# hyrise/hyrise

Hardware: AMD Instinct MI355X
Metric: rows/sec TableScan+JoinHash, TPC-H SF10 lineitem (higher is better)
Workload: dtype u16

## Files before the change

hyrise_amd/csrc/join.hip:

```cpp
#include "hy_device.hpp"
#include "hy_decode.hpp"
#include "hy_arithmetic.hpp"
#include "hy_scan_job.hpp"

#include <algorithm>
#include <atomic>
#include <cmath>
#include <chrono>
#include <cstring>
#include <type_traits>

namespace hy {

constexpr uint32_t JOIN_TILE = 4096;
constexpr uint32_t JOIN_THREADS = 512;
constexpr uint32_t JOIN_WAVES = JOIN_THREADS / 64;
constexpr uint32_t JOIN_WAVE_ROWS = JOIN_TILE / JOIN_WAVES;
constexpr uint32_t JOIN_ROUNDS = JOIN_WAVE_ROWS / 64;
constexpr uint32_t JOIN_STAGE = JOIN_TILE + 256;
constexpr uint32_t MAX_PARTITIONS = 256;
typedef uint32_t u32x2_t __attribute__((ext_vector_type(2)));
typedef uint32_t u32x4_t __attribute__((ext_vector_type(4)));
constexpr uint32_t PROBE_SIZE_PER_CHUNK = 65535u * 2u;
constexpr uint32_t BLOOM_BITS = 1u << 20;
// ... 2171 lines not shown

static void free_zeroed_blocks() {
  for (ZeroedBlocks& z : t_zeroed) {
    if (z.table) (void)hipFree(z.table);
    if (z.filter) (void)hipFree(z.filter);
    z = ZeroedBlocks{};
  }
}

void release_thread_join_state() {
  if (t_mailbox) (void)hipHostFree(t_mailbox);
  t_mailbox = t_mailbox_dev = nullptr;
  free_zeroed_blocks();
}

static hy_status join_mailbox(JoinMailbox** host, JoinMailbox** device) {
  if (!t_mailbox) {
    static_assert(sizeof(JoinMailbox) <= 256, "the mailbox is a 256-byte pinned block");
    HY_HIP(hipHostMalloc(reinterpret_cast<void**>(&t_mailbox), 256, hipHostMallocMapped));
    HY_HIP(hipHostGetDevicePointer(reinterpret_cast<void**>(&t_mailbox_dev), t_mailbox, 0));
  }
  std::memset(t_mailbox, 0, sizeof(JoinMailbox));
  *host = t_mailbox;
  *device = t_mailbox_dev;
  return HY_OK;
}

template <uint32_t WIDTH> struct FillGroup { static constexpr uint32_t ROWS = WIDTH == 4 ? 4 : 8; };
template <uint32_t WIDTH>
__device__ __forceinline__ void load_group_words(const SliceView& view, uint32_t first, uint32_t (&word)[FillGroup<WIDTH>::ROWS]) {
  const char* base = static_cast<const char*>(view.data);
  if constexpr (WIDTH == 4) {
    const u32x4_t v = *reinterpret_cast<const u32x4_t*>(base + size_t{first} * 4);
    word[0] = v.x; word[1] = v.y; word[2] = v.z; word[3] = v.w;
  } else if constexpr (WIDTH == 2) {
    const u32x4_t v = *reinterpret_cast<const u32x4_t*>(base + size_t{first} * 2);
    const uint32_t w[4] = {v.x, v.y, v.z, v.w};
#pragma unroll
    for (uint32_t j = 0; j < 8; ++j) word[j] = (w[j / 2] >> (16 * (j & 1))) & 0xFFFFu;
  } else {
    const u32x2_t v = *reinterpret_cast<const u32x2_t*>(base + first);
    const uint32_t w[2] = {v.x, v.y};
#pragma unroll
    for (uint32_t j = 0; j < 8; ++j) word[j] = (w[j / 4] >> (8 * (j & 3))) & 0xFFu;
  }
}

__device__ __forceinline__ int32_t view_key(const SliceView& view, uint32_t row) {
  if (view.kind == VIEW_INT32) return static_cast<const int32_t*>(view.data)[row];
  const uint32_t stored = view.kind == VIEW_FOR8 ? static_cast<const uint8_t*>(view.data)[row] : view.kind == VIEW_FOR16 ? static_cast<const uint16_t*>(view.data)[row] : static_cast<const uint32_t*>(view.data)[row];
  return static_cast<int32_t>(stored + static_cast<uint32_t>(static_cast<const int32_t*>(view.aux)[row / HY_FOR_BLOCK_SIZE]));
}

template <uint32_t WIDTH>
struct FillWords {
  static constexpr uint32_t GROUP = FillGroup<WIDTH>::ROWS, GROUPS = SLICE_ROWS / 256 / GROUP;
  uint32_t word[GROUPS][GROUP];
  int32_t front[GROUPS];
  uint32_t bias[GROUPS];
  int32_t key_before;
  bool has_before;
};

template <uint32_t WIDTH>
__device__ __forceinline__ void load_fill_words(const MaterializeArgs& a, const SliceView& view, uint32_t slice_index, uint32_t tid, FillWords<WIDTH>& w) {
  constexpr uint32_t GROUP = FillWords<WIDTH>::GROUP, GROUPS = FillWords<WIDTH>::GROUPS;
  const uint32_t row_count = view.row_count, lane = tid & 63;
#pragma unroll
  for (uint32_t i = 0; i < GROUPS; ++i) {
    const uint32_t first = (i * 256 + tid) * GROUP;
    load_group_words<WIDTH>(view, view.row_begin + (first < row_count ? first : 0), w.word[i]);
    w.front[i] = 0;
    if (lane == 0 && first > 0 && first < row_count) w.front[i] = view_key(view, view.row_begin + first - 1);
    w.bias[i] = view.kind == VIEW_INT32 ? 0u : static_cast<uint32_t>(static_cast<const int32_t*>(view.aux)[(view.row_begin + (first < row_count ? first : 0)) / HY_FOR_BLOCK_SIZE]);
  }
  w.key_before = 0;
  w.has_before = false;
  if (tid == 0) {
    for (uint32_t before = slice_index; before-- > 0;) {
      const SliceView earlier = a.views[before];
      if (earlier.row_count == 0) continue;
      w.key_before = view_key(earlier, earlier.row_begin + earlier.row_count - 1);
      w.has_before = true;
      break;
    }
  }
}

template <uint32_t WIDTH>
__device__ __forceinline__ void fill_checked_process(const MaterializeArgs& a, const SliceView& view, const FillWords<WIDTH>& w, uint32_t origin, uint32_t range, u32x2_entry_t* entries,
                                                     uint32_t* s_bits, uint32_t* s_base, int32_t* s_extent, uint32_t tid, int32_t* low_out, int32_t* high_out, uint32_t* flags_out) {
  constexpr uint32_t GROUP = FillGroup<WIDTH>::ROWS, GROUPS = SLICE_ROWS / 256 / GROUP;
  const uint32_t row_count = view.row_count, lane = tid & 63, wave = tid >> 6;
  const auto& word = w.word;
  int32_t front[GROUPS];
#pragma unroll
  for (uint32_t i = 0; i < GROUPS; ++i) front[i] = w.front[i];
  const int32_t key_before = w.key_before;
  const bool has_before = w.has_before;
  int32_t low = 0x7FFFFFFF, high = static_cast<int32_t>(0x80000000u);
  int32_t key[GROUPS][GROUP];
#pragma unroll
  for (uint32_t i = 0; i < GROUPS; ++i) {
    const uint32_t first = (i * 256 + tid) * GROUP;
    const uint32_t bias = w.bias[i];
#pragma unroll
// ... 125 lines not shown
  uint64_t low = ~0ull, high = 0, bits = 0;
  for (uint32_t i = tid; i < a.n_slices; i += 256) {
    uint64_t* record = partials + 4 * size_t{i};
    const uint64_t record_low = __hip_atomic_load(record + 0, __ATOMIC_RELAXED, __HIP_MEMORY_SCOPE_AGENT), record_high = __hip_atomic_load(record + 1, __ATOMIC_RELAXED, __HIP_MEMORY_SCOPE_AGENT);
    low = record_low < low ? record_low : low;
    high = record_high > high ? record_high : high;
    bits |= __hip_atomic_load(record + 2, __ATOMIC_RELAXED, __HIP_MEMORY_SCOPE_AGENT);
  }
#pragma unroll
  for (int d = 32; d > 0; d >>= 1) {
    bits |= __shfl_xor(bits, d, 64);
    const uint64_t other_low = __shfl_xor(low, d, 64), other_high = __shfl_xor(high, d, 64);
    low = other_low < low ? other_low : low;
    high = other_high > high ? other_high : high;
  }
  __syncthreads();
  if ((tid & 63) == 0) { s_min[tid >> 6] = low; s_max[tid >> 6] = high; atomicOr(&s_flags, static_cast<uint32_t>(bits)); }
  __syncthreads();
  if (tid != 0) return;
  for (uint32_t w = 0; w < 4; ++w) { low = s_min[w] < low ? s_min[w] : low; high = s_max[w] > high ? s_max[w] : high; }
  verdict->key_min = low ^ SIGN;
  verdict->key_max = high ^ SIGN;
  verdict->unsorted_signed = s_flags & 1u ? 1 : 0;
  verdict->equal_neighbours = s_flags & 2u ? 1 : 0;
  verdict->outside_hint = s_flags & 4u ? 1 : 0;
  verdict->done = 1;
  __threadfence_system();
}

constexpr uint32_t FW_STEP = 512;
constexpr uint32_t FW_STEPS_PER_SLICE = SLICE_ROWS / FW_STEP;
constexpr uint32_t FW_WINDOW = 2048;
static_assert(HY_FOR_BLOCK_SIZE % FW_STEP == 0, "a step lies in one FrameOfReference block");

constexpr uint32_t FW_BATCH = 4;

struct FillWaveState {
  uint64_t unsorted = 0, equal = 0, outside = 0;
  int32_t low = 0x7FFFFFFF, high = static_cast<int32_t>(0x80000000u);
  bool any_rows = false;
  int32_t carry = 0;
  bool has_carry = false;
};

template <uint32_t WIDTH>
__device__ __forceinline__ int32_t fill_step_key(const u32x4_t& a, const u32x4_t& b, uint32_t bias, uint32_t j) {
  uint32_t stored;
  if constexpr (WIDTH == 4) stored = j < 4 ? a[j] : b[j - 4];
  else if constexpr (WIDTH == 2) stored = (a[j / 2] >> (16 * (j & 1))) & 0xFFFFu;
  else stored = (a[j / 4] >> (8 * (j & 3))) & 0xFFu;
  return static_cast<int32_t>(stored + bias);
}

__device__ __forceinline__ bool key_in_front_of_step(const MaterializeArgs& a, uint32_t step, int32_t* key) {
  uint32_t slice = step / FW_STEPS_PER_SLICE;
  const uint32_t offset = (step % FW_STEPS_PER_SLICE) * FW_STEP;
  if (offset > 0) {
    const SliceView view = a.views[slice];
    if (view.row_count > 0) { *key = view_key(view, view.row_begin + (offset <= view.row_count ? offset : view.row_count) - 1); return true; }
  }
  while (slice-- > 0) {
    const SliceView earlier = a.views[slice];
    if (earlier.row_count == 0) continue;
    *key = view_key(earlier, earlier.row_begin + earlier.row_count - 1);
    return true;
  }
  return false;
}

__device__ __forceinline__ void fill_flush_window(const uint32_t* bits_window, uint32_t span, uint32_t first_word, uint32_t origin_word, uint32_t first_rank, bool first_is_leader, uint32_t lane,
                                                  u32x2_entry_t* entries, uint32_t* bloom_words, uint32_t debug) {
  uint32_t keys_before = 0;
  for (uint32_t begin = 0; begin < span; begin += 64) {
    const uint32_t i = begin + lane;
    const uint32_t bits = i < span ? bits_window[i] : 0u;
    const uint32_t count = __popc(bits);
    uint32_t inclusive = count;
#pragma unroll
    for (int d = 1; d < 64; d <<= 1) {
      const uint32_t other = __shfl_up(inclusive, d, 64);
      if (lane >= static_cast<uint32_t>(d)) inclusive += other;
    }
    const uint32_t base = first_rank + keys_before + inclusive - count;
    keys_before += __builtin_amdgcn_readlane(inclusive, 63);
    if (i >= span) continue;
    const uint32_t table_word = first_word + i;
    if (bits && bloom_words) atomicOr(bloom_words + ((table_word + origin_word) & (BLOOM_BITS / 32 - 1)), bits);
#ifdef HY_DEBUG_SWITCHES
    if (debug & 2) { if (bits == 0xDEADBEEFu && base == 0x12345678u) entries[0] = u32x2_entry_t{bits, base}; continue; }
#endif
    if (i == 0 || i + 1 == span) {
      if (bits) atomicOr(reinterpret_cast<uint32_t*>(entries + table_word), bits);
      if (bits && (i != 0 || first_is_leader)) reinterpret_cast<uint32_t*>(entries + table_word)[1] = base;
    } else {
      entries[table_word] = u32x2_entry_t{bits, bits ? base : 0u};
    }
  }
}

template <uint32_t WIDTH, uint32_t K>
__device__ __forceinline__ bool fill_process_steps(FillWaveState& w, const u32x4_t (&a)[K], const u32x4_t (&b)[K], const uint32_t (&bias)[K], const uint32_t (&rows)[K],
                                                   const uint32_t (&first_rank)[K], uint32_t lane, uint32_t origin, uint32_t range, u32x2_entry_t* entries, uint32_t* bloom_words,
                                                   uint32_t* bits_window, uint32_t debug) {
  const uint32_t origin_word = origin >> 5;
  if (rows[0] == 0) return true;
  int32_t key[K][8];
  uint32_t lane_rows[K];
  int32_t first_key = 0, last_key = 0;
#pragma unroll
  for (uint32_t k = 0; k < K; ++k) {
#pragma unroll
    for (uint32_t j = 0; j < 8; ++j) key[k][j] = fill_step_key<WIDTH>(a[k], b[k], bias[k], j);
    lane_rows[k] = lane * 8 < rows[k] ? (rows[k] - lane * 8 < 8 ? rows[k] - lane * 8 : 8) : 0;
    if (rows[k] != 0) {
      const uint32_t last_lane = (rows[k] - 1) >> 3, last_j = (rows[k] - 1) & 7;
      int32_t mine = key[k][0];
#pragma unroll
      for (uint32_t j = 1; j < 8; ++j) mine = last_j == j ? key[k][j] : mine;
      last_key = __builtin_amdgcn_readlane(mine, last_lane);
    }
    if (k == 0) first_key = __builtin_amdgcn_readfirstlane(key[0][0]);
  }
  const uint32_t first_rel = static_cast<uint32_t>(first_key) - origin, last_rel = static_cast<uint32_t>(last_key) - origin;
  const uint32_t first_word = first_rel >> 5;
  const bool windowed = first_rel <= range && last_rel <= range && last_rel >= first_rel && (last_rel >> 5) - first_word < FW_WINDOW;
  if (K > 1 && !windowed) return false;
  const uint32_t span = windowed ? (last_rel >> 5) - first_word + 1 : 0;
  if (!w.any_rows) w.low = first_key;
  w.high = last_key;
  w.any_rows = true;
  int32_t before[K];
  bool first_has_before[K];
  {
    int32_t carry = w.carry;
    bool has_carry = w.has_carry;
#pragma unroll
    for (uint32_t k = 0; k < K; ++k) {
      before[k] = __shfl_up(key[k][7], 1, 64);
      if (lane == 0) before[k] = carry;
      first_has_before[k] = lane != 0 || has_carry;
#pragma unroll
      for (uint32_t j = 0; j < 8; ++j) {
        const int32_t previous = j == 0 ? before[k] : key[k][j - 1];
        const bool checked = j < lane_rows[k] && (j != 0 || first_has_before[k]);
        w.unsorted |= __ballot(checked && key[k][j] < previous);
        w.equal |= __ballot(checked && key[k][j] == previous);
      }
      if (rows[k] != 0) {
        carry = __builtin_amdgcn_readlane(key[k][7], 63);
        has_carry = true;
      }
    }
  }
  const uint32_t carry_rel = static_cast<uint32_t>(w.carry) - origin;
  const bool first_is_leader = !w.has_carry || carry_rel > range || (carry_rel >> 5) != first_word;
  w.carry = last_key;
  w.has_carry = true;
  if (first_rel > range || last_rel > range) w.outside = 1;
#ifdef HY_DEBUG_SWITCHES
  if (debug & 8) return true;
#endif
  if (windowed) {
#ifdef HY_DEBUG_SWITCHES
    if (debug & 4) return true;
#endif
    for (uint32_t i = lane; i < span; i += 64) bits_window[i] = 0;
    __builtin_amdgcn_fence(__ATOMIC_RELEASE, "wavefront");
    __builtin_amdgcn_wave_barrier();
#pragma unroll
    for (uint32_t k = 0; k < K; ++k) {
#pragma unroll
      for (uint32_t j = 0; j < 8; ++j) {
        const uint32_t rel = static_cast<uint32_t>(key[k][j]) - origin;
        const uint32_t at = (rel >> 5) - first_word;
        if (j < lane_rows[k] && at < span) atomicOr(&bits_window[at], 1u << (rel & 31));
      }
    }
    __builtin_amdgcn_fence(__ATOMIC_RELEASE, "wavefront");
    __builtin_amdgcn_wave_barrier();
    __builtin_amdgcn_fence(__ATOMIC_ACQUIRE, "wavefront");
    fill_flush_window(bits_window, span, first_word, origin_word, first_rank[0], first_is_leader, lane, entries, bloom_words, debug);
    __builtin_amdgcn_wave_barrier();
  } else {
#pragma unroll
    for (uint32_t k = 0; k < K; ++k) {
      const uint32_t lane_rank = first_rank[k] + lane * 8;
#pragma unroll
      for (uint32_t j = 0; j < 8; ++j) {
        const uint32_t rel = static_cast<uint32_t>(key[k][j]) - origin;
        const int32_t previous = j == 0 ? before[k] : key[k][j - 1];
        const bool has_previous = j != 0 || first_has_before[k];
        w.outside |= __ballot(j < lane_rows[k] && rel > range);
        if (j < lane_rows[k] && rel <= range) {
          const uint32_t table_word = rel >> 5, bits = 1u << (rel & 31);
          atomicOr(reinterpret_cast<uint32_t*>(entries + table_word), bits);
          const uint32_t previous_rel = static_cast<uint32_t>(previous) - origin;
          if (!has_previous || previous_rel > range || (previous_rel >> 5) != table_word) reinterpret_cast<uint32_t*>(entries + table_word)[1] = lane_rank + j;
          if (bloom_words) atomicOr(bloom_words + ((table_word + origin_word) & (BLOOM_BITS / 32 - 1)), bits);
        }
      }
    }
  }
  return true;
}

template <uint32_t WIDTH>
struct FillBatch {
  u32x4_t a[FW_BATCH], b[FW_BATCH];
  uint32_t bias[FW_BATCH], rows[FW_BATCH], first_rank[FW_BATCH];
};

template <uint32_t WIDTH>
__device__ __forceinline__ void load_fill_batch(const MaterializeArgs& a, uint32_t batch_step, uint32_t end_step, uint32_t chunk_rows, uint32_t lane, FillBatch<WIDTH>& batch) {
  typedef const __attribute__((address_space(1))) u32x4_t* global_x4;
  typedef const __attribute__((address_space(1))) u32x2_t* global_x2;
  const uint32_t slice0 = batch_step / FW_STEPS_PER_SLICE;
  const SliceView view0 = a.views[slice0];
  const SliceView view1 = a.views[slice0 + 1 < a.n_slices ? slice0 + 1 : slice0];
  const uint32_t rank0 = view0.chunk * chunk_rows + view0.row_begin, rank1 = view1.chunk * chunk_rows + view1.row_begin;
#pragma unroll
  for (uint32_t k = 0; k < FW_BATCH; ++k) {
    const uint32_t step = batch_step + k;
    const bool second = step / FW_STEPS_PER_SLICE != slice0;
    const SliceView& view = second ? view1 : view0;
    const uint32_t offset = (step % FW_STEPS_PER_SLICE) * FW_STEP;
    batch.rows[k] = step < end_step && view.row_count > offset ? (view.row_count - offset < FW_STEP ? view.row_count - offset : FW_STEP) : 0;
    batch.first_rank[k] = (second ? rank1 : rank0) + offset;
    batch.a[k] = u32x4_t{0, 0, 0, 0};
    batch.b[k] = u32x4_t{0, 0, 0, 0};
    batch.bias[k] = 0;
    if (batch.rows[k] != 0) {
      const uint32_t row = view.row_begin + offset + (lane * 8 < batch.rows[k] ? lane * 8 : 0);
      const char* base = static_cast<const char*>(view.data);
      if constexpr (WIDTH == 4) {
        batch.a[k] = *(global_x4)(base + size_t{row} * 4);
        batch.b[k] = *(global_x4)(base + size_t{row} * 4 + 16);
      } else if constexpr (WIDTH == 2) {
        batch.a[k] = *(global_x4)(base + size_t{row} * 2);
      } else {
        const u32x2_t v = *(global_x2)(base + row);
        batch.a[k].x = v.x;
        batch.a[k].y = v.y;
      }
      if (view.kind != VIEW_INT32) batch.bias[k] = static_cast<uint32_t>(static_cast<const int32_t*>(view.aux)[(view.row_begin + offset) / HY_FOR_BLOCK_SIZE]);
    }
  }
}

struct FillCleaning {
  u32x4_t* first;
  u32x4_t* second;
  uint32_t first_vectors, second_vectors;
};

template <uint32_t WIDTH>
__global__ __launch_bounds__(256, 4) void rank_table_fill_waves(MaterializeArgs a, uint64_t key_min, uint64_t hint_range, u32x2_entry_t* entries, uint64_t* partials, uint32_t chunk_rows,
                                                             uint32_t batches_per_wave, uint32_t n_steps, uint32_t debug) {
  __shared__ uint32_t s_window[4][FW_WINDOW];
  __shared__ uint64_t s_min[4], s_max[4];
  __shared__ uint32_t s_flags;
  const uint32_t tid = threadIdx.x, lane = tid & 63, wave = __builtin_amdgcn_readfirstlane(tid >> 6);
  constexpr uint64_t SIGN = 1ull << 63;
  const uint32_t origin = static_cast<uint32_t>(key_min), range = static_cast<uint32_t>(hint_range);
  uint32_t* bloom_words = reinterpret_cast<uint32_t*>(a.bloom_out);
  uint32_t* bits_window = s_window[wave];
  const uint32_t steps_per_wave = batches_per_wave * FW_BATCH;
  const uint32_t first_step = (blockIdx.x * 4 + wave) * steps_per_wave;
  const uint32_t end_step = first_step + steps_per_wave < n_steps ? first_step + steps_per_wave : n_steps;
  if (tid == 0) s_flags = 0;
  FillWaveState w;
  FillBatch<WIDTH> current, ahead;
  if (first_step < end_step) {
    load_fill_batch<WIDTH>(a, first_step, end_step, chunk_rows, lane, current);
    int32_t front = 0;
    uint32_t has_front = 0;
    if (lane == 0) has_front = key_in_front_of_step(a, first_step, &front) ? 1u : 0u;
    w.carry = __builtin_amdgcn_readfirstlane(front);
    w.has_carry = __builtin_amdgcn_readfirstlane(has_front) != 0;
  }
  for (uint32_t batch_step = first_step; batch_step < end_step; batch_step += FW_BATCH) {
    if (batch_step + FW_BATCH < end_step) load_fill_batch<WIDTH>(a, batch_step + FW_BATCH, end_step, chunk_rows, lane, ahead);
    bool packed = true;
#pragma unroll
    for (uint32_t k = 1; k < FW_BATCH; ++k) packed = packed && (current.rows[k] == 0 || current.rows[k - 1] == FW_STEP);
    if (!packed || !fill_process_steps<WIDTH, FW_BATCH>(w, current.a, current.b, current.bias, current.rows, current.first_rank, lane, origin, range, entries, bloom_words, bits_window,
                                                        debug)) {
#pragma unroll
      for (uint32_t k = 0; k < FW_BATCH; ++k) {
        const u32x4_t one_a[1] = {current.a[k]}, one_b[1] = {current.b[k]};
        const uint32_t one_bias[1] = {current.bias[k]}, one_rows[1] = {current.rows[k]}, one_rank[1] = {current.first_rank[k]};
        fill_process_steps<WIDTH, 1>(w, one_a, one_b, one_bias, one_rows, one_rank, lane, origin, range, entries, bloom_words, bits_window, debug);
      }
    }
    current = ahead;
  }
  const uint64_t unsorted = w.unsorted, equal = w.equal, outside = w.outside;
  const int32_t low = w.low, high = w.high;
  const bool any_rows = w.any_rows;
  const uint32_t flags = (unsorted ? 1u : 0u) | (equal ? 2u : 0u) | (outside ? 4u : 0u);
  if (lane == 0) {
    s_min[wave] = any_rows ? static_cast<uint64_t>(static_cast<int64_t>(low)) ^ SIGN : ~0ull;
    s_max[wave] = any_rows ? static_cast<uint64_t>(static_cast<int64_t>(high)) ^ SIGN : 0;
  }
  __syncthreads();
  if (lane == 0 && flags) atomicOr(&s_flags, flags);
  __syncthreads();
  if (tid == 0) {
    uint64_t group_low = ~0ull, group_high = 0;
    for (uint32_t v = 0; v < 4; ++v) { group_low = s_min[v] < group_low ? s_min[v] : group_low; group_high = s_max[v] > group_high ? s_max[v] : group_high; }
    uint64_t* record = partials + 4 * size_t{blockIdx.x};
    record[0] = group_low;
    record[1] = group_high;
    record[2] = s_flags;
  }
}

template <typename K>
__global__ void publish_build_flags(const uint32_t* flags, const K* keys, uint64_t n, JoinMailbox* mailbox) {
  mailbox->unsorted = flags[0];
  mailbox->equal_neighbours = flags[1];
  mailbox->any_null = flags[2];
  mailbox->duplicate = flags[10];
  mailbox->key_or = *reinterpret_cast<const uint64_t*>(flags + 4);
  mailbox->unsorted_signed = flags[3];
  mailbox->key_min = *reinterpret_cast<const uint64_t*>(flags + 6) ^ (1ull << 63);
  mailbox->key_max = *reinterpret_cast<const uint64_t*>(flags + 8) ^ (1ull << 63);
  mailbox->first_key = n ? key_bits_of(keys[0]) : 0;
  mailbox->last_key = n ? key_bits_of(keys[n - 1]) : 0;
  __threadfence_system();
}

__global__ __launch_bounds__(256) void publish_dense_flags(const uint64_t* partials, MaterializeArgs a, uint32_t first_slice, uint32_t last_slice, JoinMailbox* mailbox) {
  __shared__ uint64_t s_all[4], s_low[4], s_high[4], s_bits[4];
  const uint32_t tid = threadIdx.x;
// ... 24 lines not shown
  mailbox->duplicate = 0;
  mailbox->key_or = all;
  mailbox->key_min = low ^ (1ull << 63);
  mailbox->key_max = high ^ (1ull << 63);
  const Slice first = a.slices[first_slice], last = a.slices[last_slice];
  mailbox->first_key = static_cast<uint64_t>(dense_key(a.segments[first.chunk], first.row_begin));
  mailbox->last_key = static_cast<uint64_t>(dense_key(a.segments[last.chunk], last.row_begin + last.row_count - 1));
  __threadfence_system();
}

__global__ __launch_bounds__(256) void plan_output(const uint64_t* base_elements, const uint64_t* base_pairs, const uint64_t* group_first_cell, uint32_t n_groups,
                                                   uint32_t n_tiles, uint64_t cells, uint64_t capacity, uint32_t slice_capacity, uint64_t* origin, uint32_t* slice_base,
                                                   uint64_t* slice_offsets, const uint32_t* n_uncached, JoinPlan* plan, JoinMailbox* mailbox) {
  __shared__ uint32_t s_wave[4];
  __shared__ uint32_t s_running;
  const uint32_t tid = threadIdx.x, lane = tid & 63, wave = tid >> 6;
  if (tid == 0) s_running = 0;
  __syncthreads();
  for (uint32_t begin = 0; begin < n_groups; begin += 256) {
    const uint32_t g = begin + tid;
    uint32_t slices = 0;
    if (g < n_groups) {
      const uint64_t first = group_first_cell ? group_first_cell[g] : static_cast<uint64_t>(g) * n_tiles;
      const uint64_t next = group_first_cell ? group_first_cell[g + 1] : static_cast<uint64_t>(g + 1) * n_tiles;
      const uint64_t from = base_elements[first], to = base_elements[next];
      origin[g] = from;
      if (g + 1 == n_groups) origin[n_groups] = to;
      slices = static_cast<uint32_t>((to - from + PROBE_SIZE_PER_CHUNK - 1) / PROBE_SIZE_PER_CHUNK);
    }
    const uint32_t inclusive = join_wave_inclusive_scan(slices);
    if (lane == 63) s_wave[wave] = inclusive;
    __syncthreads();
    uint32_t before = s_running;
    for (uint32_t w = 0; w < wave; ++w) before += s_wave[w];
    if (g < n_groups) slice_base[g] = before + inclusive - slices;
    __syncthreads();
    if (tid == 255) s_running = before + inclusive;
    __syncthreads();
  }
  if (tid == 0) {
    const uint64_t n_pairs = base_pairs[cells];
    const uint32_t n_slices = s_running;
    const uint32_t fits = n_pairs <= capacity && n_slices <= slice_capacity ? 1u : 0u;
    if (n_groups == 0) origin[0] = 0;
    plan->fits = fits;
    plan->n_slices = n_slices;
    if (fits && slice_offsets) slice_offsets[n_slices] = n_pairs;
    mailbox->n_pairs = n_pairs;
    mailbox->n_slices = n_slices;
    mailbox->n_uncached = n_uncached ? *n_uncached : 0;
    mailbox->fits = fits;
    __threadfence_system();
  }
}

__device__ __forceinline__ SliceView uniform_view(const SliceView* view) {
  typedef __attribute__((address_space(4))) const uint64_t constant_u64;
  const uint64_t address = reinterpret_cast<uint64_t>(view);
  constant_u64* q = (constant_u64*)(static_cast<uint64_t>(static_cast<uint32_t>(__builtin_amdgcn_readfirstlane(static_cast<int>(address >> 32)))) << 32 |
                                    static_cast<uint32_t>(__builtin_amdgcn_readfirstlane(static_cast<int>(address))));
  const uint64_t w0 = q[0], w1 = q[1], w2 = q[2], w3 = q[3];
  SliceView v;
  v.data = reinterpret_cast<const void*>(w0);
  v.aux = reinterpret_cast<const void*>(w1);
  v.chunk = static_cast<uint32_t>(w2);
  v.row_begin = static_cast<uint32_t>(w2 >> 32);
  v.row_count = static_cast<uint32_t>(w3);
  v.kind = static_cast<uint32_t>(w3 >> 32);
  return v;
}

#include "join_pkfk.hpp"

__global__ void publish_join_status(hy_join_status* status, uint64_t n_pairs, uint32_t n_slices, uint32_t fits) {
  status->n_pairs = n_pairs;
  status->n_slices = n_slices;
  status->fits = fits;
  status->build_confirmed = 1;
  status->error = 0;
  status->reserved = 0;
}

struct StageClock {
  bool on = HY_DEBUG_ENV("HY_JOIN_TIMING") != nullptr;
  std::chrono::steady_clock::time_point start = std::chrono::steady_clock::now();
  void mark(const char* what) {
    if (on) fprintf(stderr, "  join %-28s %8.1f us\n", what, std::chrono::duration<double, std::micro>(std::chrono::steady_clock::now() - start).count());
  }
};

static uint32_t device_cu_count();
static bool lds_atomics_are_lane_ordered(hipStream_t stream);

struct BuildSide {
  DeviceBuffer keys, rows, keys_tmp, rows_tmp, dir, bloom, flags, rank_entries, partials;
  FillCleaning cleaning{nullptr, nullptr, 0, 0};
  ZeroedBlocks* cleaned = nullptr;
  bool hint_allows_duplicates = false;
  bool bloom_is_bits = false;
  bool hinted = false;
  uint64_t hint_min = 0, hint_max = 0;
  const BuildVerdict* verdict = nullptr;
  const uint64_t* fill_records = nullptr;
  uint32_t n_fill_records = 0;
  uint64_t n = 0;
  Directory directory{};
  RankTable rank{};
  bool any_null = false;
};

static hy_status prepare_build(const hy_column* build, bool keep_nulls, bool want_bloom, bool want_ids32, uint32_t hashed_type, bool allow_rank_table, bool existence_only,
                               bool bit_filter_ok, BuildSide& b, hipStream_t stream) {
  const uint32_t n_slices = build->n_slices;
  DeviceBuffer counts, offsets;
  HY_TRY(counts.alloc(4 * size_t{n_slices + 1}));
  HY_TRY(offsets.alloc(8 * size_t{n_slices + 2}));
  HY_TRY(b.flags.alloc(64));
  bool dense = hashed_type == 0;
  for (uint32_t c = 0; c < build->n_chunks && dense; ++c) {
    const hy_segment& seg = build->host_segments[c];
    dense = (seg.encoding == HY_ENC_UNENCODED || seg.encoding == HY_ENC_FRAME_OF_REFERENCE) && seg.nulls == nullptr;
  }
// ... 1207 lines not shown
```

hyrise_amd/csrc/join_pkfk.hpp:

```cpp
#pragma once

#ifndef HY_PK_TILE
#define HY_PK_TILE 8192
#endif
#ifndef HY_PK_WAVES_PER_SIMD
#define HY_PK_WAVES_PER_SIMD 4
#endif
constexpr uint32_t PK_TILE = HY_PK_TILE;
constexpr uint32_t PK_TILES_PER_SLICE = SLICE_ROWS / PK_TILE;
constexpr uint32_t PK_ROUNDS = 16;
constexpr uint32_t PK_THREADS = PK_TILE / PK_ROUNDS;
constexpr uint32_t PK_WAVES = PK_THREADS / 64;
constexpr uint32_t PK_WAVE_ROWS = PK_TILE / PK_WAVES;
constexpr uint32_t PK_COUNT_WAVE_ROWS = 2048;
constexpr uint32_t PK_COUNT_THREADS = 64 * (PK_TILE / PK_COUNT_WAVE_ROWS);
constexpr uint32_t PK_COUNT_BATCHES = PK_COUNT_WAVE_ROWS / 512;
constexpr uint32_t PK_SCAN_THREADS = 512;
constexpr uint32_t PK_SCAN_CHUNK = 8192;
static_assert(SLICE_ROWS % PK_TILE == 0 && HY_FOR_BLOCK_SIZE % PK_WAVE_ROWS == 0 && HY_FOR_BLOCK_SIZE == PK_COUNT_WAVE_ROWS && PK_TILE % PK_COUNT_WAVE_ROWS == 0,
              "a wave's rows must lie in one FrameOfReference block");
static_assert(PK_TILE <= (1u << 13), "a staged pair keeps its row in 13 bits");

struct PkArgs {
  const SliceView* views;
// ... 242 lines not shown
  uint32_t* s_cells = pk_lds + pk_lds_presence_words(a.rank.range);
  const uint32_t tid = threadIdx.x, lane = tid & 63;
  const uint32_t sub = __builtin_amdgcn_readfirstlane(tid >> 8), wave = __builtin_amdgcn_readfirstlane((tid >> 6) & 3), local = tid & 255;
  const uint32_t partitions = 1u << a.radix_bits;
  if (blockIdx.x == 0 && tid == 0) *a.ticket = 0;
  const uint32_t words = static_cast<uint32_t>(a.rank.range >> 5) + 1;
  for (uint32_t i = tid; i < words; i += 1024) s_presence[i] = a.rank.entries[i].x;
  uint32_t* cells = s_cells + sub * partitions * COUNT_COPIES;
  for (uint32_t first = blockIdx.x * PK_LDS_SUBTILES; first < a.n_tiles; first += gridDim.x * PK_LDS_SUBTILES) {
    const uint32_t tile = first + sub;
    for (uint32_t i = local; i < partitions * COUNT_COPIES; i += 256) cells[i] = 0;
    __syncthreads();
    if (tile < a.n_tiles) {
      const SliceView view = pk_tile_view(a, tile);
      uint8_t* masks = a.row_masks + static_cast<size_t>(tile) * (2 * PK_TILE / 8);
      if (wave * PK_COUNT_WAVE_ROWS >= view.row_count) {
        for (uint32_t i = lane; i < PK_COUNT_WAVE_ROWS / 8; i += 64) { masks[wave * PK_COUNT_WAVE_ROWS / 8 + i] = 0; masks[PK_TILE / 8 + wave * PK_COUNT_WAVE_ROWS / 8 + i] = 0; }
      } else if (view.kind == VIEW_FOR8) pk_count_wave<1, true>(a, view, wave, lane, cells, s_presence, masks);
      else if (view.kind == VIEW_FOR16) pk_count_wave<2, true>(a, view, wave, lane, cells, s_presence, masks);
      else pk_count_wave<4, true>(a, view, wave, lane, cells, s_presence, masks);
    }
    __syncthreads();
    if (tile < a.n_tiles) {
      for (uint32_t partition = local; partition < partitions; partition += 256) {
        const u32x4_t low = *reinterpret_cast<const u32x4_t*>(cells + partition * COUNT_COPIES), high = *reinterpret_cast<const u32x4_t*>(cells + partition * COUNT_COPIES + 4);
        a.counts[static_cast<size_t>(partition) * a.stride + tile] = low.x + low.y + low.z + low.w + high.x + high.y + high.z + high.w;
      }
    }
    __syncthreads();
  }
}

__device__ __forceinline__ uint64_t pk_wave_inclusive_scan64(uint64_t v, uint32_t lane) {
#pragma unroll
  for (int d = 1; d < 64; d <<= 1) {
    const uint64_t other = __shfl_up(v, d, 64);
    if (lane >= static_cast<uint32_t>(d)) v += other;
  }
  return v;
}

__device__ __forceinline__ uint64_t pk_block_exclusive_scan64(uint64_t v, uint64_t* s_tmp, uint32_t tid, uint64_t* total) {
  const uint32_t lane = tid & 63, wave = tid >> 6;
  const uint64_t inclusive = pk_wave_inclusive_scan64(v, lane);
  __syncthreads();
  if (lane == 63) s_tmp[wave] = inclusive;
  __syncthreads();
  uint64_t before = 0, all = 0;
  for (uint32_t w = 0; w < PK_SCAN_THREADS / 64; ++w) { if (w < wave) before += s_tmp[w]; all += s_tmp[w]; }
  *total = all;
  return before + inclusive - v;
}

__device__ void pk_plan(const PkArgs& a, uint64_t* s_tmp, uint32_t tid) {
  const uint32_t partitions = 1u << a.radix_bits;
  uint64_t n_pairs = 0;
  uint32_t n_slices = 0;
  if (a.radix_bits) {
    const uint64_t elements = tid < partitions ? __hip_atomic_load(a.totals + tid, __ATOMIC_RELAXED, __HIP_MEMORY_SCOPE_AGENT) : 0;
    const uint64_t pairs = tid < partitions ? __hip_atomic_load(a.totals + partitions + tid, __ATOMIC_RELAXED, __HIP_MEMORY_SCOPE_AGENT) : 0;
    uint64_t total = 0;
    const uint64_t pairs_before = pk_block_exclusive_scan64(pairs, s_tmp, tid, &total);
    n_pairs = total;
    const uint64_t slices = (elements + PROBE_SIZE_PER_CHUNK - 1) / PROBE_SIZE_PER_CHUNK;
    const uint64_t slices_before = pk_block_exclusive_scan64(slices, s_tmp, tid, &total);
    n_slices = static_cast<uint32_t>(total);
    if (tid < partitions) {
      a.origin_pairs[tid] = pairs_before;
      a.slice_base[tid] = static_cast<uint32_t>(slices_before);
    }
    if (tid == 0) { a.origin_pairs[partitions] = n_pairs; a.slice_base[partitions] = n_slices; }
  } else {
    n_pairs = __hip_atomic_load(a.totals + 1, __ATOMIC_RELAXED, __HIP_MEMORY_SCOPE_AGENT);
    uint64_t running = 0;
    for (uint32_t begin = 0; begin < a.n_groups; begin += PK_SCAN_THREADS) {
      const uint32_t g = begin + tid;
      uint64_t slices = 0;
      if (g < a.n_groups) {
        const uint32_t elements = a.rel_elements[a.group_first_tile[g + 1] * PK_TILES_PER_SLICE] - a.rel_elements[a.group_first_tile[g] * PK_TILES_PER_SLICE];
        slices = (elements + PROBE_SIZE_PER_CHUNK - 1) / PROBE_SIZE_PER_CHUNK;
      }
      uint64_t total = 0;
      const uint64_t before = pk_block_exclusive_scan64(slices, s_tmp, tid, &total);
      if (g < a.n_groups) a.slice_base[g] = static_cast<uint32_t>(running + before);
      running += total;
    }
    n_slices = static_cast<uint32_t>(running);
    if (tid == 0) { a.origin_pairs[0] = 0; a.origin_pairs[1] = n_pairs; a.slice_base[a.n_groups] = n_slices; }
  }
  uint64_t build_low = ~0ull, build_high = 0, build_flags = 0;
  if (a.fill_records) {
    for (uint32_t i = tid; i < a.n_fill_records; i += PK_SCAN_THREADS) {
      const uint64_t* record = a.fill_records + 4 * size_t{i};
      build_low = record[0] < build_low ? record[0] : build_low;
      build_high = record[1] > build_high ? record[1] : build_high;
      build_flags |= record[2];
    }
#pragma unroll
    for (int d = 32; d > 0; d >>= 1) {
      build_flags |= __shfl_xor(build_flags, d, 64);
      const uint64_t other_low = __shfl_xor(build_low, d, 64), other_high = __shfl_xor(build_high, d, 64);
      build_low = other_low < build_low ? other_low : build_low;
      build_high = other_high > build_high ? other_high : build_high;
    }
    __syncthreads();
    if ((tid & 63) == 0) { s_tmp[tid >> 6] = build_low; s_tmp[8 + (tid >> 6)] = build_high; s_tmp[16 + (tid >> 6)] = build_flags; }
    __syncthreads();
  }
  if (tid == 0) {
    bool confirmed = true;
    if (a.fill_records) {
      for (uint32_t v = 0; v < PK_SCAN_THREADS / 64; ++v) {
        build_low = s_tmp[v] < build_low ? s_tmp[v] : build_low;
        build_high = s_tmp[8 + v] > build_high ? s_tmp[8 + v] : build_high;
        build_flags |= s_tmp[16 + v];
      }
      constexpr uint64_t SIGN = 1ull << 63;
      confirmed = !(build_flags & 1) && (!(build_flags & 2) || a.hint_allows_duplicates) && !(build_flags & 4) && (build_low ^ SIGN) == a.hint_min && (build_high ^ SIGN) == a.hint_max;
    } else if (a.verdict) {
      const BuildVerdict v = *a.verdict;
      confirmed = v.done && !v.unsorted_signed && (!v.equal_neighbours || a.hint_allows_duplicates) && !v.outside_hint && v.key_min == a.hint_min && v.key_max == a.hint_max;
    }
    const uint32_t fits = confirmed && n_pairs <= a.capacity && n_slices <= a.slice_capacity ? 1u : 0u;
    a.plan->fits = fits;
    a.plan->n_slices = n_slices;
    if (fits && a.slice_offsets) a.slice_offsets[n_slices] = n_pairs;
    if (a.status) {
      a.status->n_pairs = n_pairs;
      a.status->n_slices = n_slices;
      a.status->fits = fits;
      a.status->build_confirmed = confirmed ? 1u : 0u;
      a.status->error = 0;
      a.status->reserved = 0;
    } else {
      a.mailbox->n_pairs = n_pairs;
      a.mailbox->n_slices = n_slices;
      a.mailbox->n_uncached = 0;
      a.mailbox->fits = fits;
      a.mailbox->build_unconfirmed = confirmed ? 0u : 1u;
      __threadfence_system();
    }
  }
}

__global__ __launch_bounds__(PK_SCAN_THREADS) void pk_scan(PkArgs a) {
  constexpr uint32_t PER_THREAD = PK_SCAN_CHUNK / PK_SCAN_THREADS, PADDED = PK_SCAN_CHUNK + PK_SCAN_CHUNK / PER_THREAD;
  __shared__ uint32_t s_elements[PADDED], s_pairs[PADDED];
  __shared__ uint64_t s_tmp[24];
  __shared__ uint32_t s_last;
  const uint32_t tid = threadIdx.x, partition = blockIdx.x;
  const uint32_t* counts = a.counts + static_cast<size_t>(partition) * a.stride;
  uint32_t* rel_elements = a.rel_elements + static_cast<size_t>(partition) * a.stride;
  uint32_t* rel_pairs = a.rel_pairs + static_cast<size_t>(partition) * a.stride;
  uint64_t carry = 0;
  for (uint32_t begin = 0; begin < a.n_tiles; begin += PK_SCAN_CHUNK) {
    const uint32_t m = a.n_tiles - begin < PK_SCAN_CHUNK ? a.n_tiles - begin : PK_SCAN_CHUNK;
    for (uint32_t i = tid; i < PK_SCAN_CHUNK; i += PK_SCAN_THREADS) {
      const uint32_t packed = i < m ? counts[begin + i] : 0u;
      s_elements[i + i / PER_THREAD] = packed & 0xFFFFu;
      s_pairs[i + i / PER_THREAD] = packed >> 16;
    }
    __syncthreads();
    uint32_t* mine_elements = s_elements + tid * (PER_THREAD + 1);
    uint32_t* mine_pairs = s_pairs + tid * (PER_THREAD + 1);
    uint64_t sum = 0;
#pragma unroll
    for (uint32_t j = 0; j < PER_THREAD; ++j) sum += static_cast<uint64_t>(mine_elements[j]) | static_cast<uint64_t>(mine_pairs[j]) << 32;
    uint64_t total = 0;
    uint64_t run = carry + pk_block_exclusive_scan64(sum, s_tmp, tid, &total);
#pragma unroll
    for (uint32_t j = 0; j < PER_THREAD; ++j) {
      const uint64_t v = static_cast<uint64_t>(mine_elements[j]) | static_cast<uint64_t>(mine_pairs[j]) << 32;
      mine_elements[j] = static_cast<uint32_t>(run);
      mine_pairs[j] = static_cast<uint32_t>(run >> 32);
      run += v;
    }
    __syncthreads();
    for (uint32_t i = tid; i < m; i += PK_SCAN_THREADS) {
      rel_elements[begin + i] = s_elements[i + i / PER_THREAD];
      rel_pairs[begin + i] = s_pairs[i + i / PER_THREAD];
    }
    carry += total;
    __syncthreads();
  }
  if (tid == 0) {
    rel_elements[a.n_tiles] = static_cast<uint32_t>(carry);
    rel_pairs[a.n_tiles] = static_cast<uint32_t>(carry >> 32);
    __hip_atomic_store(a.totals + partition, static_cast<uint32_t>(carry), __ATOMIC_RELAXED, __HIP_MEMORY_SCOPE_AGENT);
    __hip_atomic_store(a.totals + gridDim.x + partition, static_cast<uint32_t>(carry >> 32), __ATOMIC_RELAXED, __HIP_MEMORY_SCOPE_AGENT);
    asm volatile("s_waitcnt vmcnt(0)" ::: "memory");
    const uint32_t arrived = __hip_atomic_fetch_add(a.ticket, 1u, __ATOMIC_RELAXED, __HIP_MEMORY_SCOPE_AGENT);
    s_last = arrived + 1 == gridDim.x ? 1u : 0u;
  }
  __syncthreads();
  if (!s_last) return;
  pk_plan(a, s_tmp, tid);
}

template <uint32_t WIDTH>
struct PkWords { u32x4_t piece[WIDTH]; };
template <uint32_t WIDTH>
__device__ __forceinline__ void pk_load_words(const SliceView& view, uint32_t wave, uint32_t lane, PkWords<WIDTH>& words) {
  const uint32_t first = wave * PK_WAVE_ROWS + lane * PK_ROUNDS;
  const char* base = static_cast<const char*>(view.data) + static_cast<size_t>(view.row_begin + first) * WIDTH;
  constexpr uint32_t rows_per_piece = 16 / WIDTH;
#pragma unroll
  for (uint32_t p = 0; p < WIDTH; ++p) {
    words.piece[p] = u32x4_t{0, 0, 0, 0};
    typedef const __attribute__((address_space(1))) u32x4_t* global_words;
    if (first + p * rows_per_piece < view.row_count) words.piece[p] = *(global_words)(base + p * 16);
  }
}

template <uint32_t WIDTH>
__device__ __forceinline__ void pk_words_to_block(const PkWords<WIDTH>& words, uint32_t* block, uint32_t lane) {
  u32x4_t* mine = reinterpret_cast<u32x4_t*>(reinterpret_cast<char*>(block) + lane * PK_ROUNDS * WIDTH);
#pragma unroll
  for (uint32_t p = 0; p < WIDTH; ++p) mine[p] = words.piece[p];
  __builtin_amdgcn_fence(__ATOMIC_RELEASE, "wavefront");
  __builtin_amdgcn_wave_barrier();
  __builtin_amdgcn_fence(__ATOMIC_ACQUIRE, "wavefront");
}

template <uint32_t WIDTH>
__device__ __forceinline__ uint32_t pk_block_word(const uint32_t* block, uint32_t lane, uint32_t k) {
  if constexpr (WIDTH == 2) return reinterpret_cast<const uint16_t*>(block)[k * 64 + lane];
  else if constexpr (WIDTH == 1) return reinterpret_cast<const uint8_t*>(block)[k * 64 + lane];
  else return block[k * 64 + lane];
}

typedef __attribute__((address_space(3))) uint32_t pk_lds_word;
__device__ __forceinline__ uint32_t pk_lds_address(uint32_t* word) { return static_cast<uint32_t>(reinterpret_cast<uintptr_t>((pk_lds_word*)word)); }
__device__ __forceinline__ pk_lds_word* pk_lds_pointer(uint32_t address) { return reinterpret_cast<pk_lds_word*>(static_cast<uintptr_t>(address)); }
struct PkStageTarget { uint32_t counters, spare, null_partners; };

__device__ __forceinline__ bool pk_bit(uint32_t word, uint32_t position) { return __builtin_amdgcn_ubfe(word, position, 1u) != 0; }
__device__ __forceinline__ uint32_t pk_bits_below(uint32_t word, uint32_t position) { return __popc(__builtin_amdgcn_ubfe(word, 0u, position)); }

template <bool INNER, bool STAGE>
__device__ __forceinline__ uint32_t pk_row_meta(const PkArgs& a, uint32_t key, uint32_t mask, bool valid, bool found, uint32_t k, PkStageTarget& target) {
  bool null_partner;
  const bool emit = pk_emits<INNER>(a.mode, found, &null_partner);
  if constexpr (STAGE) {
    if constexpr (!INNER) target.null_partners |= null_partner ? 1u << k : 0u;
    return (INNER ? found : valid && emit) ? target.counters + 4 * (key & mask) : target.spare;
  } else {
    return valid ? (key & mask) | (null_partner ? 0x200u : 0u) | (emit ? 0x400u : 0u) : INVALID_PARTITION;
  }
}
// ... 368 lines not shown
```

Before: 364.9 billion.

## Streamline fill kernel view loads, ascending fast path, and prefetch fill records in pk_scan

Several changes to the join build path. Slice views are now read through scalar constant loads and prefetched one batch ahead, which drops per-lane reloads and the two-view selection inside load_fill_batch. Full windowed batches get an ascending-order fast path that checks sortedness with one ballot pass and skips the bounds-checked bit setting. In pk_scan, every block now issues its fill-record loads early and reduces them before the ticket, which takes that serialized work off the last-block plan at the cost of redundant loads in every block.

```diff
diff --git a/hyrise_amd/csrc/join.hip b/hyrise_amd/csrc/join.hip
--- a/hyrise_amd/csrc/join.hip
+++ b/hyrise_amd/csrc/join.hip
@@ -2247,6 +2247,22 @@
   return static_cast<int32_t>(stored + static_cast<uint32_t>(static_cast<const int32_t*>(view.aux)[row / HY_FOR_BLOCK_SIZE]));
 }
 
+__device__ __forceinline__ SliceView uniform_view(const SliceView* view) {
+  typedef __attribute__((address_space(4))) const uint64_t constant_u64;
+  const uint64_t address = reinterpret_cast<uint64_t>(view);
+  constant_u64* q = (constant_u64*)(static_cast<uint64_t>(static_cast<uint32_t>(__builtin_amdgcn_readfirstlane(static_cast<int>(address >> 32)))) << 32 |
+                                    static_cast<uint32_t>(__builtin_amdgcn_readfirstlane(static_cast<int>(address))));
+  const uint64_t w0 = q[0], w1 = q[1], w2 = q[2], w3 = q[3];
+  SliceView v;
+  v.data = reinterpret_cast<const void*>(w0);
+  v.aux = reinterpret_cast<const void*>(w1);
+  v.chunk = static_cast<uint32_t>(w2);
+  v.row_begin = static_cast<uint32_t>(w2 >> 32);
+  v.row_count = static_cast<uint32_t>(w3);
+  v.kind = static_cast<uint32_t>(w3 >> 32);
+  return v;
+}
+
 template <uint32_t WIDTH>
 struct FillWords {
   static constexpr uint32_t GROUP = FillGroup<WIDTH>::ROWS, GROUPS = SLICE_ROWS / 256 / GROUP;
@@ -2478,20 +2494,27 @@
   return static_cast<int32_t>(stored + bias);
 }
 
-__device__ __forceinline__ bool key_in_front_of_step(const MaterializeArgs& a, uint32_t step, int32_t* key) {
+__device__ __forceinline__ bool key_in_front_of_step(const MaterializeArgs& a, uint32_t step, const SliceView& own, const SliceView& earlier, int32_t* key) {
+  typedef __attribute__((address_space(4))) const uint32_t constant_word;
   uint32_t slice = step / FW_STEPS_PER_SLICE;
   const uint32_t offset = (step % FW_STEPS_PER_SLICE) * FW_STEP;
-  if (offset > 0) {
-    const SliceView view = a.views[slice];
-    if (view.row_count > 0) { *key = view_key(view, view.row_begin + (offset <= view.row_count ? offset : view.row_count) - 1); return true; }
-  }
-  while (slice-- > 0) {
-    const SliceView earlier = a.views[slice];
-    if (earlier.row_count == 0) continue;
-    *key = view_key(earlier, earlier.row_begin + earlier.row_count - 1);
-    return true;
-  }
-  return false;
+  SliceView view = own;
+  uint32_t rows_in_front = offset <= own.row_count ? offset : own.row_count;
+  if (rows_in_front == 0 && slice > 0) {
+    --slice;
+    view = earlier;
+    rows_in_front = view.row_count;
+    while (rows_in_front == 0 && slice > 0) {
+      view = uniform_view(a.views + --slice);
+      rows_in_front = view.row_count;
+    }
+  }
+  if (rows_in_front == 0) return false;
+  const uint32_t row = view.row_begin + rows_in_front - 1;
+  if (view.kind == VIEW_INT32) { *key = static_cast<const int32_t*>(view.data)[row]; return true; }
+  const uint32_t stored = view.kind == VIEW_FOR8 ? static_cast<const uint8_t*>(view.data)[row] : view.kind == VIEW_FOR16 ? static_cast<const uint16_t*>(view.data)[row] : static_cast<const uint32_t*>(view.data)[row];
+  *key = static_cast<int32_t>(stored + ((constant_word*)view.aux)[row / HY_FOR_BLOCK_SIZE]);
+  return true;
 }
 
 __device__ __forceinline__ void fill_flush_window(const uint32_t* bits_window, uint32_t span, uint32_t first_word, uint32_t origin_word, uint32_t first_rank, bool first_is_leader, uint32_t lane,
@@ -2538,7 +2561,9 @@
 #pragma unroll
     for (uint32_t j = 0; j < 8; ++j) key[k][j] = fill_step_key<WIDTH>(a[k], b[k], bias[k], j);
     lane_rows[k] = lane * 8 < rows[k] ? (rows[k] - lane * 8 < 8 ? rows[k] - lane * 8 : 8) : 0;
-    if (rows[k] != 0) {
+    if (rows[k] == FW_STEP) {
+      last_key = __builtin_amdgcn_readlane(key[k][7], 63);
+    } else if (rows[k] != 0) {
       const uint32_t last_lane = (rows[k] - 1) >> 3, last_j = (rows[k] - 1) & 7;
       int32_t mine = key[k][0];
 #pragma unroll
@@ -2555,9 +2580,30 @@
   if (!w.any_rows) w.low = first_key;
   w.high = last_key;
   w.any_rows = true;
-  int32_t before[K];
-  bool first_has_before[K];
-  {
+  bool ascending = false;
+  if constexpr (K > 1) {
+    bool full = windowed;
+#pragma unroll
+    for (uint32_t k = 0; k < K; ++k) full = full && rows[k] == FW_STEP;
+    if (full) {
+      uint64_t not_above = 0;
+      int32_t carry = w.carry;
+#pragma unroll
+      for (uint32_t k = 0; k < K; ++k) {
+        const int32_t previous = __builtin_amdgcn_update_dpp(carry, key[k][7], 0x138, 0xF, 0xF, false);
+        uint64_t first_not_above = __builtin_amdgcn_ballot_w64(key[k][0] <= previous);
+        if (k == 0 && !w.has_carry) first_not_above &= ~1ull;
+        not_above |= first_not_above;
+#pragma unroll
+        for (uint32_t j = 1; j < 8; ++j) not_above |= __builtin_amdgcn_ballot_w64(key[k][j] <= key[k][j - 1]);
+        carry = __builtin_amdgcn_readlane(key[k][7], 63);
+      }
+      ascending = not_above == 0;
+    }
+  }
+  int32_t before[K] = {};
+  bool first_has_before[K] = {};
+  if (!ascending) {
     int32_t carry = w.carry;
     bool has_carry = w.has_carry;
 #pragma unroll
@@ -2593,13 +2639,24 @@
     for (uint32_t i = lane; i < span; i += 64) bits_window[i] = 0;
     __builtin_amdgcn_fence(__ATOMIC_RELEASE, "wavefront");
     __builtin_amdgcn_wave_barrier();
-#pragma unroll
-    for (uint32_t k = 0; k < K; ++k) {
-#pragma unroll
-      for (uint32_t j = 0; j < 8; ++j) {
-        const uint32_t rel = static_cast<uint32_t>(key[k][j]) - origin;
-        const uint32_t at = (rel >> 5) - first_word;
-        if (j < lane_rows[k] && at < span) atomicOr(&bits_window[at], 1u << (rel & 31));
+    if (ascending) {
+#pragma unroll
+      for (uint32_t k = 0; k < K; ++k) {
+#pragma unroll
+        for (uint32_t j = 0; j < 8; ++j) {
+          const uint32_t rel = static_cast<uint32_t>(key[k][j]) - origin;
+          atomicOr(&bits_window[(rel >> 5) - first_word], 1u << (rel & 31));
+        }
+      }
+    } else {
+#pragma unroll
+      for (uint32_t k = 0; k < K; ++k) {
+#pragma unroll
+        for (uint32_t j = 0; j < 8; ++j) {
+          const uint32_t rel = static_cast<uint32_t>(key[k][j]) - origin;
+          const uint32_t at = (rel >> 5) - first_word;
+          if (j < lane_rows[k] && at < span) atomicOr(&bits_window[at], 1u << (rel & 31));
+        }
       }
     }
     __builtin_amdgcn_fence(__ATOMIC_RELEASE, "wavefront");
@@ -2636,22 +2693,19 @@
   uint32_t bias[FW_BATCH], rows[FW_BATCH], first_rank[FW_BATCH];
 };
 
+static_assert(FW_STEPS_PER_SLICE % FW_BATCH == 0, "a batch lies in one slice");
 template <uint32_t WIDTH>
-__device__ __forceinline__ void load_fill_batch(const MaterializeArgs& a, uint32_t batch_step, uint32_t end_step, uint32_t chunk_rows, uint32_t lane, FillBatch<WIDTH>& batch) {
+__device__ __forceinline__ void load_fill_batch(const SliceView& view, uint32_t batch_step, uint32_t end_step, uint32_t chunk_rows, uint32_t lane, FillBatch<WIDTH>& batch) {
   typedef const __attribute__((address_space(1))) u32x4_t* global_x4;
   typedef const __attribute__((address_space(1))) u32x2_t* global_x2;
-  const uint32_t slice0 = batch_step / FW_STEPS_PER_SLICE;
-  const SliceView view0 = a.views[slice0];
-  const SliceView view1 = a.views[slice0 + 1 < a.n_slices ? slice0 + 1 : slice0];
-  const uint32_t rank0 = view0.chunk * chunk_rows + view0.row_begin, rank1 = view1.chunk * chunk_rows + view1.row_begin;
+  typedef __attribute__((address_space(4))) const uint32_t constant_word;
+  const uint32_t rank0 = view.chunk * chunk_rows + view.row_begin;
 #pragma unroll
   for (uint32_t k = 0; k < FW_BATCH; ++k) {
     const uint32_t step = batch_step + k;
-    const bool second = step / FW_STEPS_PER_SLICE != slice0;
-    const SliceView& view = second ? view1 : view0;
     const uint32_t offset = (step % FW_STEPS_PER_SLICE) * FW_STEP;
     batch.rows[k] = step < end_step && view.row_count > offset ? (view.row_count - offset < FW_STEP ? view.row_count - offset : FW_STEP) : 0;
-    batch.first_rank[k] = (second ? rank1 : rank0) + offset;
+    batch.first_rank[k] = rank0 + offset;
     batch.a[k] = u32x4_t{0, 0, 0, 0};
     batch.b[k] = u32x4_t{0, 0, 0, 0};
     batch.bias[k] = 0;
@@ -2668,7 +2722,7 @@
         batch.a[k].x = v.x;
         batch.a[k].y = v.y;
       }
-      if (view.kind != VIEW_INT32) batch.bias[k] = static_cast<uint32_t>(static_cast<const int32_t*>(view.aux)[(view.row_begin + offset) / HY_FOR_BLOCK_SIZE]);
+      if (view.kind != VIEW_INT32) batch.bias[k] = ((constant_word*)view.aux)[(view.row_begin + offset) / HY_FOR_BLOCK_SIZE];
     }
   }
 }
@@ -2696,16 +2750,27 @@
   if (tid == 0) s_flags = 0;
   FillWaveState w;
   FillBatch<WIDTH> current, ahead;
+  const uint32_t last_slice = a.n_slices - 1;
+  SliceView view_ahead = uniform_view(a.views);
+  int32_t front = 0;
+  bool has_front = false;
   if (first_step < end_step) {
-    load_fill_batch<WIDTH>(a, first_step, end_step, chunk_rows, lane, current);
-    int32_t front = 0;
-    uint32_t has_front = 0;
-    if (lane == 0) has_front = key_in_front_of_step(a, first_step, &front) ? 1u : 0u;
-    w.carry = __builtin_amdgcn_readfirstlane(front);
-    w.has_carry = __builtin_amdgcn_readfirstlane(has_front) != 0;
+    const uint32_t slice = first_step / FW_STEPS_PER_SLICE, slice_ahead = (first_step + FW_BATCH) / FW_STEPS_PER_SLICE;
+    const SliceView own = uniform_view(a.views + slice), earlier = uniform_view(a.views + (slice ? slice - 1 : 0));
+    view_ahead = uniform_view(a.views + (slice_ahead < last_slice ? slice_ahead : last_slice));
+    has_front = key_in_front_of_step(a, first_step, own, earlier, &front);
+    load_fill_batch<WIDTH>(own, first_step, end_step, chunk_rows, lane, current);
   }
   for (uint32_t batch_step = first_step; batch_step < end_step; batch_step += FW_BATCH) {
-    if (batch_step + FW_BATCH < end_step) load_fill_batch<WIDTH>(a, batch_step + FW_BATCH, end_step, chunk_rows, lane, ahead);
+    if (batch_step + FW_BATCH < end_step) {
+      load_fill_batch<WIDTH>(view_ahead, batch_step + FW_BATCH, end_step, chunk_rows, lane, ahead);
+      const uint32_t slice_ahead = (batch_step + 2 * FW_BATCH) / FW_STEPS_PER_SLICE;
+      view_ahead = uniform_view(a.views + (slice_ahead < last_slice ? slice_ahead : last_slice));
+    }
+    if (batch_step == first_step) {
+      w.carry = __builtin_amdgcn_readfirstlane(front);
+      w.has_carry = has_front;
+    }
     bool packed = true;
 #pragma unroll
     for (uint32_t k = 1; k < FW_BATCH; ++k) packed = packed && (current.rows[k] == 0 || current.rows[k - 1] == FW_STEP);
@@ -2836,22 +2901,6 @@
     mailbox->fits = fits;
     __threadfence_system();
   }
-}
-
-__device__ __forceinline__ SliceView uniform_view(const SliceView* view) {
-  typedef __attribute__((address_space(4))) const uint64_t constant_u64;
-  const uint64_t address = reinterpret_cast<uint64_t>(view);
-  constant_u64* q = (constant_u64*)(static_cast<uint64_t>(static_cast<uint32_t>(__builtin_amdgcn_readfirstlane(static_cast<int>(address >> 32)))) << 32 |
-                                    static_cast<uint32_t>(__builtin_amdgcn_readfirstlane(static_cast<int>(address))));
-  const uint64_t w0 = q[0], w1 = q[1], w2 = q[2], w3 = q[3];
-  SliceView v;
-  v.data = reinterpret_cast<const void*>(w0);
-  v.aux = reinterpret_cast<const void*>(w1);
-  v.chunk = static_cast<uint32_t>(w2);
-  v.row_begin = static_cast<uint32_t>(w2 >> 32);
-  v.row_count = static_cast<uint32_t>(w3);
-  v.kind = static_cast<uint32_t>(w3 >> 32);
-  return v;
 }
 
 #include "join_pkfk.hpp"
diff --git a/hyrise_amd/csrc/join_pkfk.hpp b/hyrise_amd/csrc/join_pkfk.hpp
--- a/hyrise_amd/csrc/join_pkfk.hpp
+++ b/hyrise_amd/csrc/join_pkfk.hpp
@@ -318,7 +318,40 @@
   return before + inclusive - v;
 }
 
-__device__ void pk_plan(const PkArgs& a, uint64_t* s_tmp, uint32_t tid) {
+struct PkFillRecords { uint64_t low[2] = {~0ull, ~0ull}, high[2] = {0, 0}, flags[2] = {0, 0}; };
+__device__ __forceinline__ void pk_request_fill_records(const PkArgs& a, uint32_t tid, PkFillRecords& r) {
+  if (!a.fill_records) return;
+#pragma unroll
+  for (uint32_t slot = 0; slot < 2; ++slot) {
+    const uint32_t i = tid + slot * PK_SCAN_THREADS;
+    if (i < a.n_fill_records) {
+      const uint64_t* record = a.fill_records + 4 * size_t{i};
+      r.low[slot] = record[0];
+      r.high[slot] = record[1];
+      r.flags[slot] = record[2];
+    }
+  }
+  for (uint32_t i = tid + 2 * PK_SCAN_THREADS; i < a.n_fill_records; i += PK_SCAN_THREADS) {
+    const uint64_t* record = a.fill_records + 4 * size_t{i};
+    r.low[0] = record[0] < r.low[0] ? record[0] : r.low[0];
+    r.high[0] = record[1] > r.high[0] ? record[1] : r.high[0];
+    r.flags[0] |= record[2];
+  }
+}
+__device__ __forceinline__ void pk_reduce_fill_records(const PkArgs& a, const PkFillRecords& r, uint64_t* s_build, uint32_t tid) {
+  if (!a.fill_records) return;
+  uint64_t build_low = r.low[0] < r.low[1] ? r.low[0] : r.low[1], build_high = r.high[0] > r.high[1] ? r.high[0] : r.high[1], build_flags = r.flags[0] | r.flags[1];
+#pragma unroll
+  for (int d = 32; d > 0; d >>= 1) {
+    build_flags |= __shfl_xor(build_flags, d, 64);
+    const uint64_t other_low = __shfl_xor(build_low, d, 64), other_high = __shfl_xor(build_high, d, 64);
+    build_low = other_low < build_low ? other_low : build_low;
+    build_high = other_high > build_high ? other_high : build_high;
+  }
+  if ((tid & 63) == 0) { s_build[tid >> 6] = build_low; s_build[8 + (tid >> 6)] = build_high; s_build[16 + (tid >> 6)] = build_flags; }
+}
+
+__device__ void pk_plan(const PkArgs& a, uint64_t* s_tmp, const uint64_t* s_build, uint32_t tid) {
   const uint32_t partitions = 1u << a.radix_bits;
   uint64_t n_pairs = 0;
   uint32_t n_slices = 0;
@@ -354,32 +387,14 @@
     n_slices = static_cast<uint32_t>(running);
     if (tid == 0) { a.origin_pairs[0] = 0; a.origin_pairs[1] = n_pairs; a.slice_base[a.n_groups] = n_slices; }
   }
-  uint64_t build_low = ~0ull, build_high = 0, build_flags = 0;
-  if (a.fill_records) {
-    for (uint32_t i = tid; i < a.n_fill_records; i += PK_SCAN_THREADS) {
-      const uint64_t* record = a.fill_records + 4 * size_t{i};
-      build_low = record[0] < build_low ? record[0] : build_low;
-      build_high = record[1] > build_high ? record[1] : build_high;
-      build_flags |= record[2];
-    }
-#pragma unroll
-    for (int d = 32; d > 0; d >>= 1) {
-      build_flags |= __shfl_xor(build_flags, d, 64);
-      const uint64_t other_low = __shfl_xor(build_low, d, 64), other_high = __shfl_xor(build_high, d, 64);
-      build_low = other_low < build_low ? other_low : build_low;
-      build_high = other_high > build_high ? other_high : build_high;
-    }
-    __syncthreads();
-    if ((tid & 63) == 0) { s_tmp[tid >> 6] = build_low; s_tmp[8 + (tid >> 6)] = build_high; s_tmp[16 + (tid >> 6)] = build_flags; }
-    __syncthreads();
-  }
   if (tid == 0) {
     bool confirmed = true;
     if (a.fill_records) {
+      uint64_t build_low = ~0ull, build_high = 0, build_flags = 0;
       for (uint32_t v = 0; v < PK_SCAN_THREADS / 64; ++v) {
-        build_low = s_tmp[v] < build_low ? s_tmp[v] : build_low;
-        build_high = s_tmp[8 + v] > build_high ? s_tmp[8 + v] : build_high;
-        build_flags |= s_tmp[16 + v];
+        build_low = s_build[v] < build_low ? s_build[v] : build_low;
+        build_high = s_build[8 + v] > build_high ? s_build[8 + v] : build_high;
+        build_flags |= s_build[16 + v];
       }
       constexpr uint64_t SIGN = 1ull << 63;
       confirmed = !(build_flags & 1) && (!(build_flags & 2) || a.hint_allows_duplicates) && !(build_flags & 4) && (build_low ^ SIGN) == a.hint_min && (build_high ^ SIGN) == a.hint_max;
@@ -412,9 +427,12 @@
 __global__ __launch_bounds__(PK_SCAN_THREADS) void pk_scan(PkArgs a) {
   constexpr uint32_t PER_THREAD = PK_SCAN_CHUNK / PK_SCAN_THREADS, PADDED = PK_SCAN_CHUNK + PK_SCAN_CHUNK / PER_THREAD;
   __shared__ uint32_t s_elements[PADDED], s_pairs[PADDED];
-  __shared__ uint64_t s_tmp[24];
+  __shared__ uint64_t s_tmp[8];
+  __shared__ uint64_t s_build[24];
   __shared__ uint32_t s_last;
   const uint32_t tid = threadIdx.x, partition = blockIdx.x;
+  PkFillRecords fill_records;
+  pk_request_fill_records(a, tid, fill_records);
   const uint32_t* counts = a.counts + static_cast<size_t>(partition) * a.stride;
   uint32_t* rel_elements = a.rel_elements + static_cast<size_t>(partition) * a.stride;
   uint32_t* rel_pairs = a.rel_pairs + static_cast<size_t>(partition) * a.stride;
@@ -449,6 +467,7 @@
     carry += total;
     __syncthreads();
   }
+  pk_reduce_fill_records(a, fill_records, s_build, tid);
   if (tid == 0) {
     rel_elements[a.n_tiles] = static_cast<uint32_t>(carry);
     rel_pairs[a.n_tiles] = static_cast<uint32_t>(carry >> 32);
@@ -460,7 +479,7 @@
   }
   __syncthreads();
   if (!s_last) return;
-  pk_plan(a, s_tmp, tid);
+  pk_plan(a, s_tmp, s_build, tid);
 }
 
 template <uint32_t WIDTH>
```

After: 364.8 billion. No clear change (-0.0%).
